# sdoira/U96-SLAM

Measured on AMD Instinct MI355X. Metric: Mpix-disparities/s, higher is better.
Workload: dtype u8

## Files before the change

u96-slam_amd/csrc/sbm_api.hip:

```cpp
#include <stdio.h>
#include <stdlib.h>
#include <string.h>

#include <algorithm>
#include <mutex>
#include <new>

#include "sbm_handle.h"

using namespace sbm;
namespace sbm { thread_local char g_sad_kernel_name[96] = ""; }

extern "C" {

void sbm_params_default(sbm_params* p, int num_disparities, int block_size) {
  if (!p) return;
  memset(p, 0, sizeof(*p));
  p->prefilter_type = SBM_PREFILTER_XSOBEL;
  p->prefilter_size = 9;
  p->prefilter_cap = 31;
  p->block_size = block_size > 0 ? block_size : 21;
  p->min_disparity = 0;
  p->num_disparities = num_disparities > 0 ? num_disparities : 64;
  p->texture_threshold = 10;
// ... 114 lines not shown
        return SBM_OK;
      }
  }
  sbm_handle* h = new (std::nothrow) sbm_handle();
  if (!h) return SBM_ERR_NOMEM;
  memset(h, 0, sizeof(*h));
  h->p = *p;
  h->device = device;
  static const char* const kSgbm[] = {"sgbm_cost", "sgbm_aggregate", "sgbm_select", "sgbm_median", "sgbm_speckle", "sgbm_total"};
  static const char* const kGftt[] = {"gftt_select_eig", "gftt_select_select", "gftt_select_total"};
  static const char* const kOrb[] = {"orb_blur", "orb_desc", "orb_total"};
  static const char* const kMatch[] = {"match_knn", "match_unique", "match_total", "match_project"};
  h->sg.clock.init(kSgbm);
  h->gs.clock.init(kGftt);
  h->orb.clock.init(kOrb);
  h->mt.clock.init(kMatch);
  static const char* const kPnp[] = {"pnp_hyp", "pnp_score", "pnp_refine", "pnp_total"};
  h->pnp.clock.init(kPnp);
  static const char* const kGfttCv[] = {"gftt_cv_eig", "gftt_cv_select", "gftt_cv_total"};
  h->gc.clock.init(kGfttCv);
  static const char* const kLk[] = {"lk_pyramid", "lk_track", "lk_total"};
  h->lk.clock.init(kLk);
  static const char* const kOcc[] = {"occ_insert", "occ_fetch"};
  h->occ.clock.init(kOcc);
  DeviceScope dscope(device);
  if (dscope.enter() != hipSuccess) {
    delete h;
    return SBM_ERR_NO_DEVICE;
  }
  bool ok = hipStreamCreateWithFlags(&h->stream, hipStreamNonBlocking) == hipSuccess;
  if (!ok) {
    destroy_now(h);
    return SBM_ERR_HIP;
  }
  h->ev_ok = true;
  for (int r = 0; r < sbm_handle::kRing; r++)
    for (int i = 0; i < sbm_handle::kMarks; i++) h->ev_ok &= hipEventCreate(&h->ev[r][i]) == hipSuccess;
  *out = h;
  return SBM_OK;
}

static void sync_all_streams(sbm_handle* h) {
  if (h->stream) hipStreamSynchronize(h->stream);
  if (h->stream_in) hipStreamSynchronize(h->stream_in);
  if (h->stream_out) hipStreamSynchronize(h->stream_out);
}

void sbm_destroy(sbm_handle* h) {
  if (!h) return;
  DeviceScope dscope(h->device);
  dscope.enter();
  h->fq_pending_dst = nullptr;
  h->fq_waited = h->fq_submitted;
  sync_all_streams(h);
  {
    std::lock_guard<std::mutex> lk(g_pool_mu);
    if (g_pool_n < kPool) {
      if (scratch_bytes(h) > kPoolScratch) {
        free_buffers(h);
      }
      g_pool[g_pool_n++] = h;
      return;
    }
  }
  destroy_now(h);
}

static void destroy_now(sbm_handle* h) {
  DeviceScope dscope(h->device);
  dscope.enter();
  sync_all_streams(h);
  free_buffers(h);
  h->sg.clock.release();
  h->gs.clock.release();
  h->gc.clock.release();
  h->orb.clock.release();
  h->mt.clock.release();
  h->pnp.clock.release();
  h->lk.clock.release();
  h->occ.clock.release();
  for (int r = 0; r < sbm_handle::kRing; r++)
    for (int i = 0; i < sbm_handle::kMarks; i++)
      if (h->ev[r][i]) hipEventDestroy(h->ev[r][i]);
  for (int i = 0; i < sbm_handle::kChunks; i++) {
    if (h->ev_in[i]) hipEventDestroy(h->ev_in[i]);
    if (h->ev_done[i]) hipEventDestroy(h->ev_done[i]);
  }
  for (int k = 0; k < 4; k++) {
    if (h->ev_fq_in[k]) hipEventDestroy(h->ev_fq_in[k]);
    if (h->ev_fq_done[k]) hipEventDestroy(h->ev_fq_done[k]);
    if (h->ev_fq_out[k]) hipEventDestroy(h->ev_fq_out[k]);
  }
  if (h->stream_in) hipStreamDestroy(h->stream_in);
  if (h->stream_out) hipStreamDestroy(h->stream_out);
  if (h->stream) hipStreamDestroy(h->stream);
  delete h;
}

int sbm_set_params(sbm_handle* h, const sbm_params* p) {
  if (!h || !p) return SBM_ERR_NULL;
  h->p = *p;
  return SBM_OK;
}

int sbm_get_params(const sbm_handle* h, sbm_params* p) {
  if (!h || !p) return SBM_ERR_NULL;
  *p = h->p;
  return SBM_OK;
}

void* sbm_stream(sbm_handle* h) { return h ? (void*)h->stream : nullptr; }
int sbm_last_hip_error(const sbm_handle* h) { return h ? h->last_hip : 0; }

int sbm_synchronize(sbm_handle* h) {
  if (!h) return SBM_ERR_NULL;
  DeviceScope dscope(h->device);
  HIPCHK(h, dscope.enter());
  HIPCHK(h, hipStreamSynchronize(h->stream));
  while (h->fq_waited != h->fq_submitted) {
    const int st = sbm_wait_oldest(h);
    if (st != SBM_OK) return st;
  }
  return SBM_OK;
}

int sbm_set_profiling(sbm_handle* h, int enabled) {
  if (!h) return SBM_ERR_NULL;
  reset_profile(h, enabled);
  return SBM_OK;
}

static void valid_roi(const sbm_params& p, int W, int H, int reading, int roi[4]) {
  int full[4] = {0, 0, W, H};
  const int* r1 = (p.roi1[2] > 0 && p.roi1[3] > 0) ? p.roi1 : full;
  const int* r2 = (p.roi2[2] > 0 && p.roi2[3] > 0) ? p.roi2 : full;
  const int sw2 = p.block_size / 2, maxd = p.min_disparity + p.num_disparities - 1;
  const int xmin = std::max(r1[0], r2[0] + maxd) + sw2;
  const int xmax = std::min(r1[0] + r1[2], r2[0] + r2[2] - ((reading & kReadRoiMinusMinD) ? p.min_disparity : 0)) - sw2;
  const int ymin = std::max(r1[1], r2[1]) + sw2;
  const int ymax = std::min(r1[1] + r1[3], r2[1] + r2[3]) - sw2;
  if (xmax - xmin > 0 && ymax - ymin > 0) {
    roi[0] = xmin; roi[1] = ymin; roi[2] = xmax - xmin; roi[3] = ymax - ymin;
  } else {
    roi[0] = roi[1] = roi[2] = roi[3] = 0;
  }
}

static int ensure_scratch(sbm_handle* h, int n, int W, int H, int pitch, bool need_cost, bool need_speckle) {
  auto& s = h->bm;
  const bool fits = n <= s.n && W == s.W && H == s.H && pitch == s.pitch && s.pf_l.p;
  if (!fits) {
    HIPCHK(h, hipStreamSynchronize(h->stream));
    release_set(s);
    const size_t npix = (size_t)n * W * H, pfbytes = (size_t)n * pitch * H + 4096;
    HIPCHK(h, s.pf_l.grow(pfbytes, h->stream));
    HIPCHK(h, s.pf_r.grow(pfbytes, h->stream));
    HIPCHK(h, s.disp_pre.grow(npix * sizeof(int16_t), h->stream));
    HIPCHK(h, hipMemsetAsync(s.pf_l.p, 0, pfbytes, h->stream));
    HIPCHK(h, hipMemsetAsync(s.pf_r.p, 0, pfbytes, h->stream));
    s.n = n; s.W = W; s.H = H; s.pitch = pitch;
  }
  const size_t npix = (size_t)s.n * W * H;
  if (need_cost) HIPCHK(h, s.cost.grow(npix * sizeof(int32_t), h->stream));
  HIPCHK(h, s.lr_keys.grow(lr_keys_bytes(s.n, W, H, need_cost), h->stream));
  if (need_speckle) HIPCHK(h, s.spk.ensure(s.n, W, H, h->stream));
  return SBM_OK;
}

static inline void mark(sbm_handle* h, int i) {
  if (h->instr) hipEventRecord(h->ev[h->calls % sbm_handle::kRing][i], h->stream);
}

static void collect_profile(sbm_handle* h) {
  unsigned nrec = std::min<unsigned>(h->calls, sbm_handle::kRing), first = 0;
  if (h->profiling == 1 && h->calls > 0) { first = (h->calls - 1) % sbm_handle::kRing; nrec = 1; }
  static const int kFrom[4] = {0, 1, 2, 4}, kTo[4] = {1, 2, 4, 5};
  float acc[4] = {0, 0, 0, 0}, tot = 0.f;
  for (unsigned r = first; r < first + nrec; r++) {
    for (int i = 0; i < 4; i++) {
      float ms = 0.f;
      if (hipEventElapsedTime(&ms, h->ev[r][kFrom[i]], h->ev[r][kTo[i]]) == hipSuccess) acc[i] += ms;
    }
    float ms = 0.f;
    if (hipEventElapsedTime(&ms, h->ev[r][0], h->ev[r][5]) == hipSuccess) tot += ms;
  }
  const float inv = nrec ? 1.f / nrec : 0.f;
  h->ms_prefilter = acc[0] * inv; h->ms_sad = acc[1] * inv; h->ms_border = 0.f; h->ms_lr = acc[2] * inv;
  h->ms_speckle = acc[3] * inv; h->ms_total = tot * inv;
}

int sbm_compute_device(sbm_handle* h, int n, const void* d_left, const void* d_right, int width, int height,
                       void* d_disp, int sync) {
  if (!h || !d_left || !d_right || !d_disp) return SBM_ERR_NULL;
  if (n <= 0) return SBM_ERR_BATCH;
  int st = sbm_params_validate(&h->p, width, height);
  if (st != SBM_OK) return st;
  if (n > 32767 || height > 65535) return SBM_ERR_UNSUPPORTED;
  const sbm_params& p = h->p;
  if (p.num_disparities > 4096) return SBM_ERR_UNSUPPORTED;
  DeviceScope dscope(h->device);
  HIPCHK(h, dscope.enter());

  Geom g;
  memset(&g, 0, sizeof(g));
  g.W = width; g.H = height; g.n = n;
  g.nd = p.num_disparities; g.mindisp = p.min_disparity; g.wsz = p.block_size; g.w2 = p.block_size / 2;
  g.cap = p.prefilter_cap; g.tex = p.texture_threshold; g.uniq = p.uniqueness_ratio;
  g.filtered = (p.min_disparity - 1) * 16;
  g.lofs = std::max(g.nd - 1 + g.mindisp, 0);
  g.rofs = -std::min(g.nd - 1 + g.mindisp, 0);
  g.width1 = width - g.rofs - g.nd + 1;
  g.xend = std::min(g.width1, width - g.lofs);
  g.want_cost = p.disp12_max_diff >= 0;
  g.padl = ((g.nd + 64 + 63) / 64) * 64;
  g.pitch = ((g.padl + width + 128 + 63) / 64) * 64;
  g.plane = g.pitch * height;
  int16_t* out = (int16_t*)d_disp;

  int roi[4];
  g.reading = env_switch("SBM_CV_READING", 0);
  valid_roi(p, width, height, g.reading, roi);
  g.row0 = std::max(roi[1], 0); g.row1 = std::min(roi[1] + roi[3], height);
  g.col0 = std::max(std::min(roi[0], width), 0); g.col1 = std::max(std::min(roi[0] + roi[2], width), 0);
  const bool range_fits = !(g.lofs >= width || g.rofs >= width || g.width1 < 1);
  const bool any_rows = range_fits && roi[2] > 0 && roi[3] > 0 && g.row1 > g.row0;
  if (!any_rows) { g.row0 = g.row1 = 0; }
  const bool speckle = p.speckle_range >= 0 && p.speckle_window_size > 0;

  st = ensure_scratch(h, n, width, height, g.pitch, g.want_cost, speckle);
  if (st != SBM_OK) return st;
  h->last = g; h->have_last = true;

  const bool in_envelope = any_rows && sad_fast_supported(g);
  bool inplace = false;
  if (in_envelope) HIPCHK(h, mqsad_inplace_ok(h->stream, &inplace));
  const bool fast = in_envelope && inplace;
  int fa = 0, fb = 0;
  if (fast) {
    const int xhi = std::min(g.W - g.lofs - 1, g.W - g.rofs - g.nd);
    fa = g.w2; fb = xhi - g.w2 + 1;
    g.cost16 = 1;
    g.pfshift = sad_fast_pfshift(g);
  }
  h->last = g;
  const bool borders_visible = g.want_cost || g.col0 < g.lofs + fa || g.col1 > g.lofs + fb;
  const bool border = fast && borders_visible;
  const uint8_t* dl = (const uint8_t*)d_left;
  const uint8_t* dr = (const uint8_t*)d_right;
  uint8_t *pf_l = h->bm.pf_l.as<uint8_t>(), *pf_r = h->bm.pf_r.as<uint8_t>();
  int16_t* disp_pre = h->bm.disp_pre.as<int16_t>();
  int32_t* cost = h->bm.cost.as<int32_t>();

  h->instr = h->profiling && h->ev_ok && (h->profiling != 3 || (h->ncall & 3u) == 0);
  mark(h, 0);
  if (any_rows) {
    if (p.prefilter_type == SBM_PREFILTER_XSOBEL) {
      HIPCHK(h, launch_prefilter(dl, dr, pf_l, pf_r, g, h->stream));
    } else {
      HIPCHK(h, h->bm.vsum.grow((size_t)2 * h->bm.n * width * height * sizeof(uint16_t), h->stream));
      HIPCHK(h, launch_prefilter_norm(dl, dr, pf_l, pf_r, h->bm.vsum.as<uint16_t>(), g, p.prefilter_size, h->stream));
    }
  }
  mark(h, 1);
  if (any_rows) {
    if (fast) {
      int xa = 0, xb = 0;
      HIPCHK(h, launch_sad_fast(pf_l, pf_r, disp_pre, cost, g, &xa, &xb, border, h->stream));
      snprintf(h->last_kernel, sizeof(h->last_kernel), "%s", g_sad_kernel_name);
      if (border && !sad_fast_borders_in_launch(g)) {
        HIPCHK(h, launch_sad_wide(pf_l, pf_r, disp_pre, cost, g, 0, xa, h->stream));
        HIPCHK(h, launch_sad_wide(pf_l, pf_r, disp_pre, cost, g, xb, g.xend, h->stream));
      }
    } else if (sad_wide_supported(g) && env_switch("SBM_WIDE", 1)) {
      HIPCHK(h, launch_sad_wide(pf_l, pf_r, disp_pre, cost, g, 0, g.xend, h->stream));
      snprintf(h->last_kernel, sizeof(h->last_kernel), in_envelope ? "sad_wide_kernel [in-place accumulate unavailable]" : "sad_wide_kernel");
    } else {
      HIPCHK(h, launch_sad_generic(pf_l, pf_r, disp_pre, cost, g, 0, g.xend, h->stream));
      snprintf(h->last_kernel, sizeof(h->last_kernel), "sad_generic_kernel");
    }
  }
  mark(h, 2);
  HIPCHK(h, launch_lrcheck(disp_pre, cost, out, h->bm.lr_keys.as<unsigned long long>(), g, p.disp12_max_diff, h->stream));
  mark(h, 4);
  if (speckle)
    HIPCHK(h, launch_speckle(out, h->bm.spk, g, p.speckle_window_size, p.speckle_range, h->stream));
  mark(h, 5);
  if (h->instr) h->calls++;
  h->ncall++;
  if (sync || h->profiling == 1) HIPCHK(h, hipStreamSynchronize(h->stream));
  return SBM_OK;
}

int sbm_rect_map_device(sbm_handle* h, const sbm_rect_cam* cam, int width, int height, void* d_map, int sync) {
  if (!h || !cam || !d_map) return SBM_ERR_NULL;
  if (width <= 0 || height <= 0 || width > 32767 || height > 32767) return SBM_ERR_SIZE;
  DeviceScope dscope(h->device);
  HIPCHK(h, dscope.enter());
  HIPCHK(h, launch_rect_map(*cam, width, height, (int16_t*)d_map, h->stream));
  if (sync) HIPCHK(h, hipStreamSynchronize(h->stream));
  return SBM_OK;
}

int sbm_rect_remap_device(sbm_handle* h, int n, const void* d_src, const void* d_map, int width, int height, void* d_dst,
                          int sync) {
  if (!h || !d_src || !d_map || !d_dst) return SBM_ERR_NULL;
  if (n <= 0) return SBM_ERR_BATCH;
  if (width <= 0 || height <= 0 || width > 32767 || height > 32767) return SBM_ERR_SIZE;
  if (((size_t)width * height + 1023) / 1024 > 65535) return SBM_ERR_UNSUPPORTED;
  DeviceScope dscope(h->device);
  HIPCHK(h, dscope.enter());
  HIPCHK(h, launch_rect_remap((const uint8_t*)d_src, (const int16_t*)d_map, (uint8_t*)d_dst, n, width, height, h->stream));
  if (sync) HIPCHK(h, hipStreamSynchronize(h->stream));
  return SBM_OK;
}

int sbm_prefilter_device(sbm_handle* h, int n, const void* d_src, int width, int height, int flavour, int cap,
                         void* d_dst, int sync) {
  if (!h || !d_src || !d_dst) return SBM_ERR_NULL;
  if (n <= 0) return SBM_ERR_BATCH;
  if (width <= 0 || height <= 0) return SBM_ERR_SIZE;
  if (flavour != SBM_PREFILTER_FLAVOUR_CV && flavour != SBM_PREFILTER_FLAVOUR_RTL) return SBM_ERR_PREFILTER_TYPE;
  if (flavour == SBM_PREFILTER_FLAVOUR_CV && (cap < 1 || cap > 63)) return SBM_ERR_PREFILTER_CAP;
  if (n > 65534 || height > 65535 * 4) return SBM_ERR_UNSUPPORTED;
  DeviceScope dscope(h->device);
  HIPCHK(h, dscope.enter());
  HIPCHK(h, launch_prefilter_dense((const uint8_t*)d_src, (uint8_t*)d_dst, n, width, height,
                                   flavour == SBM_PREFILTER_FLAVOUR_RTL, cap, h->stream));
  if (sync) HIPCHK(h, hipStreamSynchronize(h->stream));
  return SBM_OK;
}

int sbm_disparity_to_float_device(sbm_handle* h, int n, const void* d_disp, int width, int height, void* d_out, int sync) {
  if (!h || !d_disp || !d_out) return SBM_ERR_NULL;
  if (n <= 0) return SBM_ERR_BATCH;
  if (width <= 0 || height <= 0) return SBM_ERR_SIZE;
  DeviceScope dscope(h->device);
  HIPCHK(h, dscope.enter());
  HIPCHK(h, launch_disp_to_float((const int16_t*)d_disp, (float*)d_out, (size_t)n * width * height, h->stream));
  if (sync) HIPCHK(h, hipStreamSynchronize(h->stream));
  return SBM_OK;
}

int sbm_decimate_device(sbm_handle* h, int n, const void* d_disp, int width, int height, int scale, void* d_out, int sync) {
  if (!h || !d_disp || !d_out) return SBM_ERR_NULL;
  if (n <= 0) return SBM_ERR_BATCH;
  if (width <= 0 || height <= 0 || scale <= 0) return SBM_ERR_SIZE;
  DeviceScope dscope(h->device);
  HIPCHK(h, dscope.enter());
  HIPCHK(h, launch_decimate((const int16_t*)d_disp, (int16_t*)d_out, n, width, height, scale, h->stream));
  if (sync) HIPCHK(h, hipStreamSynchronize(h->stream));
  return SBM_OK;
}

int sbm_reproject_device(sbm_handle* h, int n, const void* d_disp, int width, int height, int scale,
                         const sbm_stereo_model* model, int apply_local, void* d_xyz, int sync) {
  if (!h || !d_disp || !d_xyz || !model) return SBM_ERR_NULL;
  if (n <= 0) return SBM_ERR_BATCH;
  if (width <= 0 || height <= 0 || scale <= 0) return SBM_ERR_SIZE;
  DeviceScope dscope(h->device);
  HIPCHK(h, dscope.enter());
  HIPCHK(h, launch_reproject((const int16_t*)d_disp, (float*)d_xyz, n, width, height, scale, *model, apply_local, h->stream));
  if (sync) HIPCHK(h, hipStreamSynchronize(h->stream));
  return SBM_OK;
}

int sbm_keypoints3d_device(sbm_handle* h, const void* d_disp, int width, int height, const void* d_kpts, int nk,
                           const sbm_stereo_model* model, float min_depth, float max_depth, void* d_xyz, int sync) {
  if (!h || !d_disp || !model || (nk > 0 && (!d_kpts || !d_xyz))) return SBM_ERR_NULL;
  if (width <= 0 || height <= 0 || nk < 0) return SBM_ERR_SIZE;
  DeviceScope dscope(h->device);
  HIPCHK(h, dscope.enter());
  HIPCHK(h, launch_keypoints3d((const int16_t*)d_disp, (const float*)d_kpts, (float*)d_xyz, width, height, nk, *model,
                               min_depth, max_depth, h->stream));
  if (sync) HIPCHK(h, hipStreamSynchronize(h->stream));
  return SBM_OK;
}

int sbm_get_profile(sbm_handle* h, const char* name, float* ms) {
  if (!h || !name || !ms) return SBM_ERR_NULL;
  DeviceScope dscope(h->device);
  HIPCHK(h, dscope.enter());
  HIPCHK(h, hipStreamSynchronize(h->stream));
  if (h->profiling && h->ev_ok) collect_profile(h);
  if (!strcmp(name, "prefilter")) *ms = h->ms_prefilter;
  else if (!strcmp(name, "sad")) *ms = h->ms_sad;
  else if (!strcmp(name, "border")) *ms = h->ms_border;
  else if (!strcmp(name, "lrcheck")) *ms = h->ms_lr;
  else if (!strcmp(name, "speckle")) *ms = h->ms_speckle;
  else if (!strcmp(name, "total")) *ms = h->ms_total;
  else {
    const float* t = h->sg.clock.find(name);
    if (!t) t = h->gs.clock.find(name);
    if (!t) t = h->gc.clock.find(name);
    if (!t) t = h->orb.clock.find(name);
    if (!t) t = h->mt.clock.find(name);
    if (!t) t = h->pnp.clock.find(name);
    if (!t) t = h->lk.clock.find(name);
    if (!t) t = h->occ.clock.find(name);
    if (!t) return SBM_ERR_UNSUPPORTED;
    *ms = *t;
  }
  return SBM_OK;
}

int sbm_last_kernel_name(sbm_handle* h, char* dst, size_t dst_bytes) {
  if (!h || !dst || dst_bytes == 0) return SBM_ERR_NULL;
  snprintf(dst, dst_bytes, "%s", h->last_kernel);
  return SBM_OK;
}

int sbm_debug_fetch(sbm_handle* h, int which, void* dst, size_t dst_bytes) {
  if (!h || !dst) return SBM_ERR_NULL;
  if (which >= 4 && which <= 6) return sgbm_debug_fetch(h, which, dst, dst_bytes);
  if (!h->have_last) return SBM_ERR_UNSUPPORTED;
  const Geom& g = h->last;
  DeviceScope dscope(h->device);
  HIPCHK(h, dscope.enter());
  HIPCHK(h, hipStreamSynchronize(h->stream));
  const size_t npix = (size_t)g.n * g.W * g.H;
  if (which == 0 || which == 1) {
    if (dst_bytes < npix) return SBM_ERR_SIZE;
    const uint8_t* src = (which == 0 ? h->bm.pf_l : h->bm.pf_r).as<uint8_t>();
    HIPCHK(h, hipMemcpy2D(dst, g.W, src + g.padl, g.pitch, g.W, (size_t)g.n * g.H, hipMemcpyDeviceToHost));
    uint8_t* d = (uint8_t*)dst;
    for (size_t i = 0; i < npix; i++) d[i] = (uint8_t)((d[i] - kPfBias) >> g.pfshift);
    return SBM_OK;
  }
  if (which == 2) {
    if (!h->bm.cost.p) return SBM_ERR_UNSUPPORTED;
    if (dst_bytes < npix * sizeof(int32_t)) return SBM_ERR_SIZE;
    if (g.cost16) {
      uint16_t* tmp = (uint16_t*)malloc(npix * sizeof(uint16_t));
      if (!tmp) return SBM_ERR_NOMEM;
      hipError_t e = hipMemcpy(tmp, h->bm.cost.p, npix * sizeof(uint16_t), hipMemcpyDeviceToHost);
      if (e == hipSuccess)
        for (size_t i = 0; i < npix; i++) ((int32_t*)dst)[i] = tmp[i];
      free(tmp);
      HIPCHK(h, e);
      return SBM_OK;
    }
    HIPCHK(h, hipMemcpy(dst, h->bm.cost.p, npix * sizeof(int32_t), hipMemcpyDeviceToHost));
    return SBM_OK;
  }
  if (which == 3) {
    if (dst_bytes < npix * sizeof(int16_t)) return SBM_ERR_SIZE;
    HIPCHK(h, hipMemcpy(dst, h->bm.disp_pre.p, npix * sizeof(int16_t), hipMemcpyDeviceToHost));
    int16_t* d = (int16_t*)dst;
    for (int i = 0; i < g.n; i++)
      for (int y = 0; y < g.H; y++) {
        int16_t* row = d + ((size_t)i * g.H + y) * g.W;
        const bool live = y >= g.row0 && y < g.row1;
        for (int x = 0; x < g.W; x++)
          if (!live || x < g.lofs || x >= g.lofs + g.xend) row[x] = (int16_t)g.filtered;
      }
    return SBM_OK;
  }
  return SBM_ERR_UNSUPPORTED;
}

}
```

u96-slam_amd/csrc/sbm_common.h:

```cpp
#pragma once
#include <hip/hip_runtime.h>
#include <stdint.h>

#include "../../include/sbm.h"

#include <stdlib.h>

namespace sbm {

inline int env_switch(const char* name, int dflt) {
  const char* e = getenv(name);
  return e ? atoi(e) : dflt;
}

struct Geom {
  int W, H;
  int n;
  int pitch;
  int padl;
  int plane;
  int nd, mindisp, wsz, w2, cap;
  int lofs, rofs, width1, xend;
  int tex, uniq;
  int filtered;
  int row0, row1;
  int col0, col1;
  int want_cost;
  int cost16;
  int pfshift;
  int reading;
};

constexpr int kReadRoiMinusMinD = 1;
constexpr int kReadCostShort = 2;
constexpr int kReadSpeckleX16 = 4;
constexpr int kReadOddRowComputed = 8;
constexpr int kReadLrTieLater = 16;

constexpr int kPfBias = 1;

hipError_t launch_prefilter(const uint8_t* d_left, const uint8_t* d_right, uint8_t* pf_l, uint8_t* pf_r,
                            const Geom& g, hipStream_t s);

hipError_t launch_prefilter_norm(const uint8_t* d_left, const uint8_t* d_right, uint8_t* pf_l, uint8_t* pf_r, uint16_t* vsum,
                                 const Geom& g, int winsize, hipStream_t s);

hipError_t launch_sad_generic(const uint8_t* pf_l, const uint8_t* pf_r, int16_t* disp, int32_t* cost, const Geom& g,
                              int xa, int xb, hipStream_t s);

bool sad_wide_supported(const Geom& g);
hipError_t launch_sad_wide(const uint8_t* pf_l, const uint8_t* pf_r, int16_t* disp, int32_t* cost, const Geom& g, int xa, int xb,
                           hipStream_t s);

extern thread_local char g_sad_kernel_name[96];
bool sad_fast_supported(const Geom& g);
hipError_t mqsad_inplace_ok(hipStream_t s, bool* ok);
constexpr int kFastNdMax = 512;
bool sad_fast_borders_in_launch(const Geom& g);
int sad_fast_pfshift(const Geom& g);
hipError_t launch_sad_fast(const uint8_t* pf_l, const uint8_t* pf_r, int16_t* disp, int32_t* cost, const Geom& g,
                           int* xa, int* xb, bool border, hipStream_t s);

constexpr int kLrLdsCols = 8192;
inline size_t lr_keys_bytes(int n, int W, int H, bool do_lr) {
  return do_lr && W > kLrLdsCols ? (size_t)n * H * W * sizeof(unsigned long long) : 0;
}
hipError_t launch_lrcheck(const int16_t* disp_pre, const int32_t* cost, int16_t* disp_out, unsigned long long* keys,
                          const Geom& g, int disp12_max_diff, hipStream_t s);

constexpr int kSpkMaxSeg = 4, kSpkRecordPad = 288, kSpkSeamPad = 512;

hipError_t launch_prefilter_dense(const uint8_t* d_src, uint8_t* d_dst, int n, int W, int H, int rtl, int cap,
                                  hipStream_t s);
hipError_t launch_rect_map(const sbm_rect_cam& cam, int W, int H, int16_t* d_map, hipStream_t s);
hipError_t launch_rect_remap(const uint8_t* d_src, const int16_t* d_map, uint8_t* d_dst, int n, int W, int H,
                             hipStream_t s);

hipError_t launch_gftt_eig(const uint8_t* img, uint16_t* eig, unsigned* maxv, int n, int W, int H, hipStream_t s);

hipError_t launch_disp_to_float(const int16_t* disp, float* out, size_t count, hipStream_t s);
hipError_t launch_decimate(const int16_t* disp, int16_t* out, int n, int W, int H, int scale, hipStream_t s);
hipError_t launch_reproject(const int16_t* disp, float* xyz, int n, int W, int H, int scale, const sbm_stereo_model& m,
                            int apply_local, hipStream_t s);
hipError_t launch_keypoints3d(const int16_t* disp, const float* kp, float* xyz, int W, int H, int nk,
                              const sbm_stereo_model& m, float min_depth, float max_depth, hipStream_t s);
hipError_t launch_keypoints3d_lk(const float* kp, const float* rp, const uint8_t* status, const int* count, int n, int cap,
                                 const sbm_stereo_model& m, float min_depth, float max_depth, float* xyz, hipStream_t s);

struct SgbmGeom {
  int W, H, n;
  int minD, D, minX1, maxX1, W1;
  int SW2, P1, P2, ftzero, uniq, d12;
  int fullDP;
  int reading;
};

}
```

u96-slam_amd/csrc/sbm_handle.h:

```cpp
#pragma once
#include <string.h>

#include "sbm_common.h"

#define HIPCHK(h, call)                         \
  do {                                          \
    hipError_t e_ = (call);                     \
    if (e_ != hipSuccess) {                     \
      (h)->last_hip = (int)e_;                  \
      return e_ == hipErrorOutOfMemory ? SBM_ERR_NOMEM : SBM_ERR_HIP; \
    }                                           \
  } while (0)

struct DeviceScope {
  int prev, dev;
  bool have;
  explicit DeviceScope(int d) : prev(-1), dev(d), have(false) { have = hipGetDevice(&prev) == hipSuccess; }
  hipError_t enter() { return (have && prev == dev) ? hipSuccess : hipSetDevice(dev); }
  ~DeviceScope() {
    if (have && prev != dev) hipSetDevice(prev);
  }
};

namespace sbm {

struct DevBuf {
  void* p;
  size_t bytes;
  template <class T> T* as() const { return static_cast<T*>(p); }
  hipError_t grow(size_t need, hipStream_t s) {
    if (need <= bytes) return hipSuccess;
    hipError_t e = p ? hipStreamSynchronize(s) : hipSuccess;
    if (e != hipSuccess) return e;
    release();
    e = hipMalloc(&p, need);
    if (e != hipSuccess) { p = nullptr; return e; }
    bytes = need;
    return hipSuccess;
  }
  void release() { hipFree(p); p = nullptr; bytes = 0; }
};

template <class Set> void release_all(Set& s) { s.each([](DevBuf& b) { b.release(); }); }
template <class Set> size_t bytes_held(Set& s) {
  size_t n = 0;
  s.each([&](DevBuf& b) { n += b.bytes; });
  return n;
}
template <class Set> void release_set(Set& s) {
  release_all(s);
  s.n = s.W = s.H = 0;
}

struct SpeckleScratch {
  int n, W, H;
  DevBuf runs, nheads, seam, nseam;
  template <class F> void each(F f) { f(runs); f(nheads); f(seam); f(nseam); }
  static size_t bytes(int n, int W, int H, size_t* part);
  hipError_t ensure(int n_, int W_, int H_, hipStream_t s) {
    if (nseam.p && n_ <= n && W_ == W && H_ == H) return hipSuccess;
    hipError_t e = bytes_held(*this) ? hipStreamSynchronize(s) : hipSuccess;
    if (e != hipSuccess) return e;
    release_set(*this);
    size_t part[4];
    bytes(n_, W_, H_, part);
    DevBuf* b[4] = {&runs, &nheads, &seam, &nseam};
    for (int i = 0; i < 4 && e == hipSuccess; i++) e = b[i]->grow(part[i], s);
    if (e == hipSuccess) { n = n_; W = W_; H = H_; }
    return e;
  }
};

hipError_t launch_speckle(int16_t* disp, const SpeckleScratch& sc, const Geom& g, int max_size, int max_diff, hipStream_t s);

struct StageClock {
  static constexpr int kMax = 6;
  const char* const* names;
  int nstage;
  bool on;
  hipEvent_t ev[kMax];
  float ms[kMax];
  template <int N> void init(const char* const (&table)[N]) { static_assert(N <= kMax, ""); names = table; nstage = N; }
  hipError_t start(bool profiling) {
    on = profiling;
    hipError_t e = hipSuccess;
    for (int i = 0; on && i < nstage && e == hipSuccess; i++)
      if (!ev[i]) e = hipEventCreate(&ev[i]);
    if (on) reset();
    return e;
  }
  hipError_t mark(int i, hipStream_t s) { return on ? hipEventRecord(ev[i], s) : hipSuccess; }
  hipError_t add(int stage, int a, int b) {
    if (!on) return hipSuccess;
    float t = 0.f;
    hipError_t e = hipEventSynchronize(ev[b]);
    if (e == hipSuccess) e = hipEventElapsedTime(&t, ev[a], ev[b]);
    ms[stage] += t;
    return e;
  }
  void reset() { for (float& t : ms) t = 0.f; }
  void release() {
    for (hipEvent_t& e : ev)
      if (e) { hipEventDestroy(e); e = nullptr; }
  }
  const float* find(const char* name) const {
    for (int i = 0; i < nstage; i++)
      if (!strcmp(name, names[i])) return &ms[i];
    return nullptr;
  }
};

}

struct sbm_handle {
  sbm_params p;
  int device;
  hipStream_t stream;
  int last_hip;
  struct {
    int n, W, H, pitch;
    sbm::DevBuf pf_l, pf_r;
    sbm::DevBuf disp_pre;
    sbm::DevBuf cost;
    sbm::DevBuf lr_keys;
    sbm::DevBuf vsum;
    sbm::SpeckleScratch spk;
    template <class F> void each(F f) { f(pf_l); f(pf_r); f(disp_pre); f(cost); f(lr_keys); f(vsum); spk.each(f); }
  } bm;
  struct {
    int n, W, H;
    int gen;
    sbm::DevBuf rec, flag, xs_l, xs_r;
    template <class F> void each(F f) { f(rec); f(flag); f(xs_l); f(xs_r); }
  } fp;
  struct {
    int n, W, H;
    sbm::DevBuf l, r, d;
    sbm::DevBuf zc_cnt;
    template <class F> void each(F f) { f(l); f(r); f(d); f(zc_cnt); }
  } st;
  uint8_t* pin;
  size_t pin_bytes;
  int16_t* zc_out;
  size_t zc_bytes;
  unsigned* zc_flag;
  unsigned zc_seq;
  hipStream_t stream_in, stream_out;
  static constexpr int kChunks = 64;
  hipEvent_t ev_in[kChunks], ev_done[kChunks];
  bool pipe_ok;
  struct {
    int n, W, H;
    sbm::DevBuf l[2], r[2], d[2];
    template <class F> void each(F f) {
      for (int k = 0; k < 2; k++) { f(l[k]); f(r[k]); f(d[k]); }
    }
  } fq;
  hipEvent_t ev_fq_in[4], ev_fq_done[4], ev_fq_out[4];
  bool fq_ok;
  unsigned fq_submitted, fq_waited;
  int16_t* fq_pending_dst;
  size_t fq_pending_bytes;
  char last_kernel[128];
  sbm::Geom last;
  bool have_last;
  int profiling;
  unsigned ncall;
  bool instr;
  static constexpr int kRing = 64, kMarks = 6;
  hipEvent_t ev[kRing][kMarks];
  bool ev_ok;
  unsigned calls;
  float ms_prefilter, ms_sad, ms_border, ms_lr, ms_speckle, ms_total;
  struct {
    sbm::DevBuf C, S, pre;
    sbm::SpeckleScratch spk;
    sbm::SgbmGeom last;
    bool have_last, last_one_chunk;
    sbm::StageClock clock;
    template <class F> void each(F f) { f(C); f(S); f(pre); spk.each(f); }
  } sg;
  struct {
    sbm::DevBuf tab, out;
    sbm::StageClock clock;
    template <class F> void each(F f) { f(tab); f(out); }
  } gs;
  struct {
    sbm::DevBuf keys, small, eig, tab, out;
    sbm::StageClock clock;
    template <class F> void each(F f) { f(keys); f(small); f(eig); f(tab); f(out); }
  } gc;
  struct {
    sbm::DevBuf blur, io;
    sbm::StageClock clock;
    template <class F> void each(F f) { f(blur); f(io); }
  } orb;
  struct {
    sbm::DevBuf scratch, io;
    sbm::StageClock clock;
    template <class F> void each(F f) { f(scratch); f(io); }
  } mt;
  struct {
    sbm::DevBuf scratch, io;
    sbm::StageClock clock;
    template <class F> void each(F f) { f(scratch); f(io); }
  } pnp;
  struct {
    sbm::DevBuf pyr, deriv, io;
    sbm::StageClock clock;
    template <class F> void each(F f) { f(pyr); f(deriv); f(io); }
  } lk;
  struct {
    sbm::DevBuf sort, hist, io;
    sbm::StageClock clock;
    template <class F> void each(F f) { f(sort); f(hist); f(io); }
  } occ;
};

namespace sbm {

void free_staging(sbm_handle* h);
int ensure_staging(sbm_handle* h, int n, int W, int H);
int gftt_select_run(sbm_handle* h, int n, const void* d_img, const void* d_eig, const void* d_max, int width, int height,
                    const sbm_gftt_select_params* p, void* d_kpts, void* d_count, int sync);
int gftt_cv_run(sbm_handle* h, int n, const void* d_img, int width, int height, const sbm_gftt_cv_params* p, void* d_eig, void* d_max,
                void* d_kpts, void* d_count, int sync);
int sgbm_debug_fetch(sbm_handle* h, int which, void* dst, size_t dst_bytes);

}
```

u96-slam_amd/csrc/sbm_lrcheck.hip:

```cpp
#include <stdlib.h>

#include <algorithm>

#include "sbm_common.h"

namespace sbm {

struct LrArgs {
  const int16_t* disp_pre;
  const void* cost;
  int16_t* disp_out;
  int cost16;
  int W, H, mindisp, nd, tol, filtered, row0, row1, col0, col1, do_lr;
  int cx0, cx1;
  int cost_short, tie_later;
  unsigned long long* keys;
};

extern __shared__ __attribute__((aligned(16))) unsigned long long lr_keys[];

template <bool GK>
__global__ void __launch_bounds__(256) lrcheck_kernel(LrArgs a) {
  const int y = blockIdx.x;
  const size_t base = ((size_t)blockIdx.y * a.H + y) * a.W;
  int16_t* out = a.disp_out + base;
  if (y < a.row0 || y >= a.row1) {
    for (int x = threadIdx.x; x < a.W; x += 256) out[x] = (int16_t)a.filtered;
    return;
  }
  const int16_t* dp = a.disp_pre + base;
  if (!a.do_lr) {
    const int lo = max(a.col0, a.cx0), hi = min(a.col1, a.cx1);
    for (int x = threadIdx.x; x < a.W; x += 256) out[x] = (x >= lo && x < hi) ? dp[x] : (int16_t)a.filtered;
    return;
  }
  const uint16_t* cp16 = static_cast<const uint16_t*>(a.cost) + base;
  const int32_t* cp32 = static_cast<const int32_t*>(a.cost) + base;
  const int INV = a.filtered;
  const int minX1 = max(max(a.mindisp + a.nd, 0), a.cx0), maxX1 = min(a.W + min(a.mindisp, 0), a.cx1);
  unsigned long long* const keys = GK ? a.keys + base : lr_keys;
  for (int x = threadIdx.x; x < a.W; x += 256) keys[x] = ~0ull;
  if (GK) __threadfence();
  __syncthreads();
  for (int x = minX1 + threadIdx.x; x < maxX1; x += 256) {
    const int d = dp[x];
    if (d == INV) continue;
    const int x2 = x - ((d + 8) >> 4);
    if (x2 >= 0 && x2 < a.W) {
      unsigned c = a.cost16 ? (unsigned)cp16[x] : (unsigned)cp32[x];
      if (a.cost_short) c = (unsigned)((int)(short)c + 32768);
      atomicMin(&keys[x2], ((unsigned long long)c << 32) | (unsigned)(a.tie_later ? a.W - 1 - x : x));
    }
  }
  if (GK) __threadfence();
  __syncthreads();
  auto key_at = [&](int i) -> unsigned long long {
    if (GK) return __hip_atomic_load(&keys[i], __ATOMIC_RELAXED, __HIP_MEMORY_SCOPE_AGENT);
    return keys[i];
  };
  for (int x = threadIdx.x; x < a.W; x += 256) {
    int d = (x >= a.cx0 && x < a.cx1) ? dp[x] : INV;
    if (x < a.col0 || x >= a.col1) {
      d = INV;
    } else if (d != INV && x >= minX1 && x < maxX1) {
      const int xa = x - (d >> 4), xb = x - ((d + 15) >> 4);
      bool bad_a = false, bad_b = false;
      if (xa >= 0 && xa < a.W) {
        const unsigned long long k = key_at(xa);
        if (k != ~0ull) {
          const int xw = (int)(k & 0xffffffffu);
          const int d2 = dp[a.tie_later ? a.W - 1 - xw : xw];
          bad_a = abs(d2 - d) > a.tol;
        }
      }
      if (xb >= 0 && xb < a.W) {
        const unsigned long long k = key_at(xb);
        if (k != ~0ull) {
          const int xw = (int)(k & 0xffffffffu);
          const int d2 = dp[a.tie_later ? a.W - 1 - xw : xw];
          bad_b = abs(d2 - d) > a.tol;
        }
      }
      if (bad_a && bad_b) d = INV;
    }
    out[x] = (int16_t)d;
  }
}

extern __shared__ __attribute__((aligned(16))) unsigned lr_lds32[];

template <int NIT, int PX>
__global__ void __launch_bounds__(320) lrcheck16_kernel(LrArgs a) {
  const int BS = blockDim.x;
  const int y = blockIdx.x;
  const size_t base = ((size_t)blockIdx.y * a.H + y) * a.W;
  int16_t* out = a.disp_out + base;
  if (y < a.row0 || y >= a.row1) {
    for (int x = threadIdx.x; x < a.W; x += BS) out[x] = (int16_t)a.filtered;
    return;
  }
  unsigned* const key = lr_lds32;
  const int W = a.W;
  const int16_t* dp = a.disp_pre + base;
  const uint16_t* cp = static_cast<const uint16_t*>(a.cost) + base;
  const int INV = a.filtered;
  const int minX1 = max(max(a.mindisp + a.nd, 0), a.cx0), maxX1 = min(W + min(a.mindisp, 0), a.cx1);
  constexpr unsigned NONE = 0xffffffffu;
  const unsigned tol2 = 2u * (unsigned)a.tol;
  const int dbias = 0x8000 - a.tol;
  const int wbase = PX * __builtin_amdgcn_readfirstlane((int)(threadIdx.x & ~63u));
  const int lo = max(max(minX1, a.cx0), a.col0), hi = min(min(maxX1, a.cx1), min(a.col1, W));
  bool inner[NIT];
#pragma unroll
  for (int k = 0; k < NIT; k++) inner[k] = wbase + PX * BS * k >= lo && wbase + PX * BS * k + 64 * PX <= hi;
  int dv[NIT][PX];
  unsigned kv[NIT][PX];
  auto load = [&](auto inner_t, const int k) {
    constexpr bool IN = decltype(inner_t)::value;
    const int x0 = PX * (threadIdx.x + BS * k);
    unsigned dd[PX / 2], cc[PX / 2];
#pragma unroll
    for (int j = 0; j < PX / 2; j++) dd[j] = cc[j] = 0;
    if (IN || x0 + PX <= W) {
      __builtin_memcpy(dd, dp + x0, 2 * PX);
      __builtin_memcpy(cc, cp + x0, 2 * PX);
    } else {
      for (int i = 0; x0 + i < W; i++) {
        dd[i >> 1] |= (unsigned)(unsigned short)dp[x0 + i] << (16 * (i & 1));
        cc[i >> 1] |= (unsigned)cp[x0 + i] << (16 * (i & 1));
      }
    }
#pragma unroll
    for (int j = 0; j < PX / 2; j++) {
      const unsigned db = dd[j] ^ 0x80008000u;
      dv[k][2 * j] = (int)(short)(dd[j] & 0xffffu);
      dv[k][2 * j + 1] = (int)dd[j] >> 16;
      kv[k][2 * j] = __builtin_amdgcn_perm(cc[j], db, 0x05040100u);
      kv[k][2 * j + 1] = __builtin_amdgcn_perm(cc[j], db, 0x07060302u);
    }
    if (!IN) {
#pragma unroll
      for (int i = 0; i < PX; i++)
        if (!(x0 + i >= a.cx0 && x0 + i < a.cx1)) dv[k][i] = INV;
    }
  };
  const int dummy = W + 3 + (threadIdx.x & 63);
  auto claim = [&](auto inner_t, const int k) {
    constexpr bool IN = decltype(inner_t)::value;
#pragma unroll
    for (int i = 0; i < PX; i++) {
      const int x = PX * (threadIdx.x + BS * k) + i;
      const int d = dv[k][i];
      const int x2 = x - ((d + 8) >> 4);
      if (IN) {
        __hip_atomic_fetch_min(&key[x2 + 1], kv[k][i], __ATOMIC_RELAXED, __HIP_MEMORY_SCOPE_WORKGROUP);
      } else {
        const bool claims = d != INV && x >= minX1 && x < maxX1 && (unsigned)x2 < (unsigned)W;
        __hip_atomic_fetch_min(&key[claims ? x2 + 1 : dummy], kv[k][i], __ATOMIC_RELAXED, __HIP_MEMORY_SCOPE_WORKGROUP);
      }
    }
  };
  auto check = [&](auto inner_t, const int k) {
    constexpr bool IN = decltype(inner_t)::value;
    const int x0 = PX * (threadIdx.x + BS * k);
    if (!IN && x0 >= W) return;
    unsigned k0[PX], k1[PX];
#pragma unroll
    for (int i = 0; i < PX; i++) {
      const int x = x0 + i;
      const int d = dv[k][i];
      const int xa = x - (d >> 4);
      int p = xa;
      if (!IN) {
        const bool checked = ((int)(d != INV) & (int)(x >= minX1 && x < maxX1) & (int)((unsigned)xa < (unsigned)W)) != 0;
        p = checked ? xa : W + 1;
      }
      k0[i] = key[p];
      k1[i] = key[p + 1];
    }
    unsigned res[PX];
#pragma unroll
    for (int i = 0; i < PX; i++) {
      const int x = x0 + i;
      const int d = dv[k][i];
      const unsigned ka = k1[i], kb = (d & 15) ? k0[i] : k1[i];
      const unsigned dbt = (unsigned)(d + dbias);
      const unsigned ta = (ka - dbt) & 0xffffu, tb = (kb - dbt) & 0xffffu;
      const bool bad = ((int)(max(ka, kb) < 0xffff0000u) & (int)(min(ta, tb) > tol2)) != 0;
      res[i] = (unsigned)(((!IN && (x < a.col0 || x >= a.col1)) || bad) ? INV : d);
    }
    if (IN || x0 + PX <= W) {
      unsigned r2[PX / 2];
#pragma unroll
      for (int j = 0; j < PX / 2; j++) r2[j] = __builtin_amdgcn_perm(res[2 * j + 1], res[2 * j], 0x05040100u);
      __builtin_memcpy(out + x0, r2, 2 * PX);
    } else {
      for (int i = 0; x0 + i < W; i++) out[x0 + i] = (int16_t)res[i];
    }
  };
#pragma unroll
  for (int k = 0; k < NIT; k++) {
    if (inner[k]) load(std::true_type{}, k);
    else load(std::false_type{}, k);
  }
  for (int i = 4 * threadIdx.x; i < W + 3; i += 4 * BS) *reinterpret_cast<uint4*>(key + i) = make_uint4(NONE, NONE, NONE, NONE);
  __syncthreads();
#pragma unroll
  for (int k = 0; k < NIT; k++) {
    if (inner[k]) claim(std::true_type{}, k);
    else claim(std::false_type{}, k);
  }
  __syncthreads();
#pragma unroll
  for (int k = 0; k < NIT; k++) {
    if (inner[k]) check(std::true_type{}, k);
    else check(std::false_type{}, k);
  }
}

hipError_t launch_lrcheck(const int16_t* disp_pre, const int32_t* cost, int16_t* disp_out, unsigned long long* keys,
                          const Geom& g, int disp12_max_diff, hipStream_t s) {
  LrArgs a;
  a.keys = keys;
  a.disp_pre = disp_pre; a.cost = cost; a.disp_out = disp_out; a.cost16 = g.cost16;
  a.W = g.W; a.H = g.H; a.mindisp = g.mindisp; a.nd = g.nd; a.tol = disp12_max_diff * 16; a.filtered = g.filtered;
  a.row0 = g.row0; a.row1 = g.row1; a.col0 = g.col0; a.col1 = g.col1; a.do_lr = disp12_max_diff >= 0;
  a.cx0 = g.lofs; a.cx1 = g.lofs + g.xend;
  a.cost_short = (g.reading & kReadCostShort) != 0; a.tie_later = (g.reading & kReadLrTieLater) != 0;
  if (a.do_lr && g.cost16 && g.W <= 4096 && (g.nd + 1) * 16 <= 16384 && !a.cost_short && !a.tie_later) {
    a.tol = std::min(a.tol, 16384);
    const size_t lds16 = (size_t)(g.W + 3 + 64 + 8) * sizeof(unsigned);
    const int px = g.W <= 1280 ? 2 : 4;
    const int bsmax = px == 4 ? 256 : (g.W <= 640 ? 64 : 128);
    const int groups = (g.W + px - 1) / px;
    const int nit = (groups + bsmax - 1) / bsmax;
    const int bs = (((groups + nit - 1) / nit + 63) / 64) * 64;
    const dim3 grid(g.H, g.n), block(bs);
    bool launched = true;
#define SBM_LR_CASE(N, P) case N * 8 + P: hipLaunchKernelGGL((lrcheck16_kernel<N, P>), grid, block, lds16, s, a); break;
    switch (nit * 8 + px) {
      SBM_LR_CASE(1, 2) SBM_LR_CASE(2, 2) SBM_LR_CASE(3, 2) SBM_LR_CASE(4, 2) SBM_LR_CASE(5, 2)
      SBM_LR_CASE(2, 4) SBM_LR_CASE(3, 4) SBM_LR_CASE(4, 4)
      default: launched = false;
    }
#undef SBM_LR_CASE
    if (launched) return hipGetLastError();
    a.tol = disp12_max_diff * 16;
  }
  if (a.do_lr && g.W > kLrLdsCols) {
    if (!keys) return hipErrorInvalidValue;
    hipLaunchKernelGGL(lrcheck_kernel<true>, dim3(g.H, g.n), dim3(256), 0, s, a);
  } else {
    const size_t lds = a.do_lr ? (size_t)g.W * sizeof(unsigned long long) : 0;
    hipLaunchKernelGGL(lrcheck_kernel<false>, dim3(g.H, g.n), dim3(256), lds, s, a);
  }
  return hipGetLastError();
}

}
```

Before: 4.323 million.

## Compute SAD disparities directly into output and run LR check in place

Drops the intermediate disp_pre buffer. The SAD stage now writes straight into the output disparity array, and the LR-check kernels update it in place, storing only pixels whose value changes or that lie outside the computed range. For the global-atomic path, the LR key now carries the disparity itself instead of a column index, so the check no longer needs to read back another pixel that may already have been overwritten. This removes one full-frame int16 read-plus-write pass and most of the LR-stage stores. The cost is that the debug readout of pre-LR disparities now reruns the SAD stage into a separate buffer.

Result: no change. 4.359 million, median of 6 (+0.8%).

```diff
diff --git a/u96-slam_amd/csrc/sbm_api.hip b/u96-slam_amd/csrc/sbm_api.hip
--- a/u96-slam_amd/csrc/sbm_api.hip
+++ b/u96-slam_amd/csrc/sbm_api.hip
@@ -290,10 +290,9 @@
   if (!fits) {
     HIPCHK(h, hipStreamSynchronize(h->stream));
     release_set(s);
-    const size_t npix = (size_t)n * W * H, pfbytes = (size_t)n * pitch * H + 4096;
+    const size_t pfbytes = (size_t)n * pitch * H + 4096;
     HIPCHK(h, s.pf_l.grow(pfbytes, h->stream));
     HIPCHK(h, s.pf_r.grow(pfbytes, h->stream));
-    HIPCHK(h, s.disp_pre.grow(npix * sizeof(int16_t), h->stream));
     HIPCHK(h, hipMemsetAsync(s.pf_l.p, 0, pfbytes, h->stream));
     HIPCHK(h, hipMemsetAsync(s.pf_r.p, 0, pfbytes, h->stream));
     s.n = n; s.W = W; s.H = H; s.pitch = pitch;
@@ -325,6 +324,27 @@
   const float inv = nrec ? 1.f / nrec : 0.f;
   h->ms_prefilter = acc[0] * inv; h->ms_sad = acc[1] * inv; h->ms_border = 0.f; h->ms_lr = acc[2] * inv;
   h->ms_speckle = acc[3] * inv; h->ms_total = tot * inv;
+}
+
+static int run_sad(sbm_handle* h, const Geom& g, int16_t* disp) {
+  uint8_t *pf_l = h->bm.pf_l.as<uint8_t>(), *pf_r = h->bm.pf_r.as<uint8_t>();
+  int32_t* cost = h->bm.cost.as<int32_t>();
+  if (h->last_fast) {
+    int xa = 0, xb = 0;
+    HIPCHK(h, launch_sad_fast(pf_l, pf_r, disp, cost, g, &xa, &xb, h->last_border, h->stream));
+    snprintf(h->last_kernel, sizeof(h->last_kernel), "%s", g_sad_kernel_name);
+    if (h->last_border && !sad_fast_borders_in_launch(g)) {
+      HIPCHK(h, launch_sad_wide(pf_l, pf_r, disp, cost, g, 0, xa, h->stream));
+      HIPCHK(h, launch_sad_wide(pf_l, pf_r, disp, cost, g, xb, g.xend, h->stream));
+    }
+  } else if (sad_wide_supported(g) && env_switch("SBM_WIDE", 1)) {
+    HIPCHK(h, launch_sad_wide(pf_l, pf_r, disp, cost, g, 0, g.xend, h->stream));
+    snprintf(h->last_kernel, sizeof(h->last_kernel), h->last_in_envelope ? "sad_wide_kernel [in-place accumulate unavailable]" : "sad_wide_kernel");
+  } else {
+    HIPCHK(h, launch_sad_generic(pf_l, pf_r, disp, cost, g, 0, g.xend, h->stream));
+    snprintf(h->last_kernel, sizeof(h->last_kernel), "sad_generic_kernel");
+  }
+  return SBM_OK;
 }
 
 int sbm_compute_device(sbm_handle* h, int n, const void* d_left, const void* d_right, int width, int height,
@@ -386,8 +406,7 @@
   const uint8_t* dl = (const uint8_t*)d_left;
   const uint8_t* dr = (const uint8_t*)d_right;
   uint8_t *pf_l = h->bm.pf_l.as<uint8_t>(), *pf_r = h->bm.pf_r.as<uint8_t>();
-  int16_t* disp_pre = h->bm.disp_pre.as<int16_t>();
-  int32_t* cost = h->bm.cost.as<int32_t>();
+  h->last_any_rows = any_rows; h->last_fast = fast; h->last_border = border; h->last_in_envelope = in_envelope;
 
   h->instr = h->profiling && h->ev_ok && (h->profiling != 3 || (h->ncall & 3u) == 0);
   mark(h, 0);
@@ -401,24 +420,11 @@
   }
   mark(h, 1);
   if (any_rows) {
-    if (fast) {
-      int xa = 0, xb = 0;
-      HIPCHK(h, launch_sad_fast(pf_l, pf_r, disp_pre, cost, g, &xa, &xb, border, h->stream));
-      snprintf(h->last_kernel, sizeof(h->last_kernel), "%s", g_sad_kernel_name);
-      if (border && !sad_fast_borders_in_launch(g)) {
-        HIPCHK(h, launch_sad_wide(pf_l, pf_r, disp_pre, cost, g, 0, xa, h->stream));
-        HIPCHK(h, launch_sad_wide(pf_l, pf_r, disp_pre, cost, g, xb, g.xend, h->stream));
-      }
-    } else if (sad_wide_supported(g) && env_switch("SBM_WIDE", 1)) {
-      HIPCHK(h, launch_sad_wide(pf_l, pf_r, disp_pre, cost, g, 0, g.xend, h->stream));
-      snprintf(h->last_kernel, sizeof(h->last_kernel), in_envelope ? "sad_wide_kernel [in-place accumulate unavailable]" : "sad_wide_kernel");
-    } else {
-      HIPCHK(h, launch_sad_generic(pf_l, pf_r, disp_pre, cost, g, 0, g.xend, h->stream));
-      snprintf(h->last_kernel, sizeof(h->last_kernel), "sad_generic_kernel");
-    }
+    st = run_sad(h, g, out);
+    if (st != SBM_OK) return st;
   }
   mark(h, 2);
-  HIPCHK(h, launch_lrcheck(disp_pre, cost, out, h->bm.lr_keys.as<unsigned long long>(), g, p.disp12_max_diff, h->stream));
+  HIPCHK(h, launch_lrcheck(out, h->bm.cost.as<int32_t>(), h->bm.lr_keys.as<unsigned long long>(), g, p.disp12_max_diff, h->stream));
   mark(h, 4);
   if (speckle)
     HIPCHK(h, launch_speckle(out, h->bm.spk, g, p.speckle_window_size, p.speckle_range, h->stream));
@@ -582,12 +588,18 @@
   }
   if (which == 3) {
     if (dst_bytes < npix * sizeof(int16_t)) return SBM_ERR_SIZE;
-    HIPCHK(h, hipMemcpy(dst, h->bm.disp_pre.p, npix * sizeof(int16_t), hipMemcpyDeviceToHost));
+    if (h->last_any_rows) {
+      HIPCHK(h, h->bm.dbg_pre.grow(npix * sizeof(int16_t), h->stream));
+      const int st = run_sad(h, g, h->bm.dbg_pre.as<int16_t>());
+      if (st != SBM_OK) return st;
+      HIPCHK(h, hipStreamSynchronize(h->stream));
+      HIPCHK(h, hipMemcpy(dst, h->bm.dbg_pre.p, npix * sizeof(int16_t), hipMemcpyDeviceToHost));
+    }
     int16_t* d = (int16_t*)dst;
     for (int i = 0; i < g.n; i++)
       for (int y = 0; y < g.H; y++) {
         int16_t* row = d + ((size_t)i * g.H + y) * g.W;
-        const bool live = y >= g.row0 && y < g.row1;
+        const bool live = h->last_any_rows && y >= g.row0 && y < g.row1;
         for (int x = 0; x < g.W; x++)
           if (!live || x < g.lofs || x >= g.lofs + g.xend) row[x] = (int16_t)g.filtered;
       }
diff --git a/u96-slam_amd/csrc/sbm_common.h b/u96-slam_amd/csrc/sbm_common.h
--- a/u96-slam_amd/csrc/sbm_common.h
+++ b/u96-slam_amd/csrc/sbm_common.h
@@ -65,8 +65,8 @@
 inline size_t lr_keys_bytes(int n, int W, int H, bool do_lr) {
   return do_lr && W > kLrLdsCols ? (size_t)n * H * W * sizeof(unsigned long long) : 0;
 }
-hipError_t launch_lrcheck(const int16_t* disp_pre, const int32_t* cost, int16_t* disp_out, unsigned long long* keys,
-                          const Geom& g, int disp12_max_diff, hipStream_t s);
+hipError_t launch_lrcheck(int16_t* disp, const int32_t* cost, unsigned long long* keys, const Geom& g, int disp12_max_diff,
+                          hipStream_t s);
 
 constexpr int kSpkMaxSeg = 4, kSpkRecordPad = 288, kSpkSeamPad = 512;
 
diff --git a/u96-slam_amd/csrc/sbm_handle.h b/u96-slam_amd/csrc/sbm_handle.h
--- a/u96-slam_amd/csrc/sbm_handle.h
+++ b/u96-slam_amd/csrc/sbm_handle.h
@@ -120,12 +120,12 @@
   struct {
     int n, W, H, pitch;
     sbm::DevBuf pf_l, pf_r;
-    sbm::DevBuf disp_pre;
+    sbm::DevBuf dbg_pre;
     sbm::DevBuf cost;
     sbm::DevBuf lr_keys;
     sbm::DevBuf vsum;
     sbm::SpeckleScratch spk;
-    template <class F> void each(F f) { f(pf_l); f(pf_r); f(disp_pre); f(cost); f(lr_keys); f(vsum); spk.each(f); }
+    template <class F> void each(F f) { f(pf_l); f(pf_r); f(dbg_pre); f(cost); f(lr_keys); f(vsum); spk.each(f); }
   } bm;
   struct {
     int n, W, H;
@@ -164,6 +164,7 @@
   char last_kernel[128];
   sbm::Geom last;
   bool have_last;
+  bool last_any_rows, last_fast, last_border, last_in_envelope;
   int profiling;
   unsigned ncall;
   bool instr;
diff --git a/u96-slam_amd/csrc/sbm_lrcheck.hip b/u96-slam_amd/csrc/sbm_lrcheck.hip
--- a/u96-slam_amd/csrc/sbm_lrcheck.hip
+++ b/u96-slam_amd/csrc/sbm_lrcheck.hip
@@ -7,9 +7,8 @@
 namespace sbm {
 
 struct LrArgs {
-  const int16_t* disp_pre;
+  int16_t* disp;
   const void* cost;
-  int16_t* disp_out;
   int cost16;
   int W, H, mindisp, nd, tol, filtered, row0, row1, col0, col1, do_lr;
   int cx0, cx1;
@@ -23,15 +22,16 @@
 __global__ void __launch_bounds__(256) lrcheck_kernel(LrArgs a) {
   const int y = blockIdx.x;
   const size_t base = ((size_t)blockIdx.y * a.H + y) * a.W;
-  int16_t* out = a.disp_out + base;
+  int16_t* out = a.disp + base;
   if (y < a.row0 || y >= a.row1) {
     for (int x = threadIdx.x; x < a.W; x += 256) out[x] = (int16_t)a.filtered;
     return;
   }
-  const int16_t* dp = a.disp_pre + base;
+  const int16_t* dp = out;
   if (!a.do_lr) {
     const int lo = max(a.col0, a.cx0), hi = min(a.col1, a.cx1);
-    for (int x = threadIdx.x; x < a.W; x += 256) out[x] = (x >= lo && x < hi) ? dp[x] : (int16_t)a.filtered;
+    for (int x = threadIdx.x; x < a.W; x += 256)
+      if (!(x >= lo && x < hi)) out[x] = (int16_t)a.filtered;
     return;
   }
   const uint16_t* cp16 = static_cast<const uint16_t*>(a.cost) + base;
@@ -49,7 +49,8 @@
     if (x2 >= 0 && x2 < a.W) {
       unsigned c = a.cost16 ? (unsigned)cp16[x] : (unsigned)cp32[x];
       if (a.cost_short) c = (unsigned)((int)(short)c + 32768);
-      atomicMin(&keys[x2], ((unsigned long long)c << 32) | (unsigned)(a.tie_later ? a.W - 1 - x : x));
+      const unsigned dk = (unsigned)(d ^ 0x8000) & 0xffffu;
+      atomicMin(&keys[x2], ((unsigned long long)c << 32) | (a.tie_later ? 0xffffu - dk : dk));
     }
   }
   if (GK) __threadfence();
@@ -58,8 +59,14 @@
     if (GK) return __hip_atomic_load(&keys[i], __ATOMIC_RELAXED, __HIP_MEMORY_SCOPE_AGENT);
     return keys[i];
   };
+  auto key_disp = [&](unsigned long long k) -> int {
+    const unsigned dk = (unsigned)k & 0xffffu;
+    return (int)(short)((a.tie_later ? 0xffffu - dk : dk) ^ 0x8000u);
+  };
   for (int x = threadIdx.x; x < a.W; x += 256) {
-    int d = (x >= a.cx0 && x < a.cx1) ? dp[x] : INV;
+    const bool computed = x >= a.cx0 && x < a.cx1;
+    const int d0 = computed ? dp[x] : INV;
+    int d = d0;
     if (x < a.col0 || x >= a.col1) {
       d = INV;
     } else if (d != INV && x >= minX1 && x < maxX1) {
@@ -67,23 +74,15 @@
       bool bad_a = false, bad_b = false;
       if (xa >= 0 && xa < a.W) {
         const unsigned long long k = key_at(xa);
-        if (k != ~0ull) {
-          const int xw = (int)(k & 0xffffffffu);
-          const int d2 = dp[a.tie_later ? a.W - 1 - xw : xw];
-          bad_a = abs(d2 - d) > a.tol;
-        }
+        if (k != ~0ull) bad_a = abs(key_disp(k) - d) > a.tol;
       }
       if (xb >= 0 && xb < a.W) {
         const unsigned long long k = key_at(xb);
-        if (k != ~0ull) {
-          const int xw = (int)(k & 0xffffffffu);
-          const int d2 = dp[a.tie_later ? a.W - 1 - xw : xw];
-          bad_b = abs(d2 - d) > a.tol;
-        }
+        if (k != ~0ull) bad_b = abs(key_disp(k) - d) > a.tol;
       }
       if (bad_a && bad_b) d = INV;
     }
-    out[x] = (int16_t)d;
+    if (!computed || d != d0) out[x] = (int16_t)d;
   }
 }
 
@@ -94,14 +93,14 @@
   const int BS = blockDim.x;
   const int y = blockIdx.x;
   const size_t base = ((size_t)blockIdx.y * a.H + y) * a.W;
-  int16_t* out = a.disp_out + base;
+  int16_t* out = a.disp + base;
   if (y < a.row0 || y >= a.row1) {
     for (int x = threadIdx.x; x < a.W; x += BS) out[x] = (int16_t)a.filtered;
     return;
   }
   unsigned* const key = lr_lds32;
   const int W = a.W;
-  const int16_t* dp = a.disp_pre + base;
+  const int16_t* dp = out;
   const uint16_t* cp = static_cast<const uint16_t*>(a.cost) + base;
   const int INV = a.filtered;
   const int minX1 = max(max(a.mindisp + a.nd, 0), a.cx0), maxX1 = min(W + min(a.mindisp, 0), a.cx1);
@@ -115,6 +114,7 @@
   for (int k = 0; k < NIT; k++) inner[k] = wbase + PX * BS * k >= lo && wbase + PX * BS * k + 64 * PX <= hi;
   int dv[NIT][PX];
   unsigned kv[NIT][PX];
+  unsigned force = 0u;
   auto load = [&](auto inner_t, const int k) {
     constexpr bool IN = decltype(inner_t)::value;
     const int x0 = PX * (threadIdx.x + BS * k);
@@ -141,7 +141,7 @@
     if (!IN) {
 #pragma unroll
       for (int i = 0; i < PX; i++)
-        if (!(x0 + i >= a.cx0 && x0 + i < a.cx1)) dv[k][i] = INV;
+        if (!(x0 + i >= a.cx0 && x0 + i < a.cx1)) { dv[k][i] = INV; force |= 1u << (PX * k + i); }
     }
   };
   const int dummy = W + 3 + (threadIdx.x & 63);
@@ -179,6 +179,7 @@
       k1[i] = key[p + 1];
     }
     unsigned res[PX];
+    bool store[PX], any = false;
 #pragma unroll
     for (int i = 0; i < PX; i++) {
       const int x = x0 + i;
@@ -188,14 +189,19 @@
       const unsigned ta = (ka - dbt) & 0xffffu, tb = (kb - dbt) & 0xffffu;
       const bool bad = ((int)(max(ka, kb) < 0xffff0000u) & (int)(min(ta, tb) > tol2)) != 0;
       res[i] = (unsigned)(((!IN && (x < a.col0 || x >= a.col1)) || bad) ? INV : d);
+      store[i] = (int)res[i] != d || (!IN && ((force >> (PX * k + i)) & 1u));
+      any |= store[i];
     }
     if (IN || x0 + PX <= W) {
-      unsigned r2[PX / 2];
-#pragma unroll
-      for (int j = 0; j < PX / 2; j++) r2[j] = __builtin_amdgcn_perm(res[2 * j + 1], res[2 * j], 0x05040100u);
-      __builtin_memcpy(out + x0, r2, 2 * PX);
+      if (any) {
+        unsigned r2[PX / 2];
+#pragma unroll
+        for (int j = 0; j < PX / 2; j++) r2[j] = __builtin_amdgcn_perm(res[2 * j + 1], res[2 * j], 0x05040100u);
+        __builtin_memcpy(out + x0, r2, 2 * PX);
+      }
     } else {
-      for (int i = 0; x0 + i < W; i++) out[x0 + i] = (int16_t)res[i];
+      for (int i = 0; x0 + i < W; i++)
+        if (store[i]) out[x0 + i] = (int16_t)res[i];
     }
   };
 #pragma unroll
@@ -218,11 +224,11 @@
   }
 }
 
-hipError_t launch_lrcheck(const int16_t* disp_pre, const int32_t* cost, int16_t* disp_out, unsigned long long* keys,
-                          const Geom& g, int disp12_max_diff, hipStream_t s) {
+hipError_t launch_lrcheck(int16_t* disp, const int32_t* cost, unsigned long long* keys, const Geom& g, int disp12_max_diff,
+                          hipStream_t s) {
   LrArgs a;
   a.keys = keys;
-  a.disp_pre = disp_pre; a.cost = cost; a.disp_out = disp_out; a.cost16 = g.cost16;
+  a.disp = disp; a.cost = cost; a.cost16 = g.cost16;
   a.W = g.W; a.H = g.H; a.mindisp = g.mindisp; a.nd = g.nd; a.tol = disp12_max_diff * 16; a.filtered = g.filtered;
   a.row0 = g.row0; a.row1 = g.row1; a.col0 = g.col0; a.col1 = g.col1; a.do_lr = disp12_max_diff >= 0;
   a.cx0 = g.lofs; a.cx1 = g.lofs + g.xend;
```
